# pablopalafox/semantic-depth

Hardware: AMD Instinct MI355X
Metric: fused frames/sec (FCN-8s+monodepth+pcl fusion) at 512x1024 (higher is better)
Workload: dtype fp32-grade: f32 operands as fp16 hi + 2^11-scaled lo planes (22 bits), 3 fp16 MFMA products, f32 accumulate; 1 GPU; BASELINE.json configs[3]: full fused pipeline (seg + depth + pcl back-projection + road width), batch 32 per GPU, 512x1024, monodepth-resnet50 on frame+flip, seeded synthetic weights; survey_config=4, engine=f16x2, approach=rw, overlap=True, full=False, found=32

## Files before the change

### semantic_depth_amd/csrc/dec_tail.hip

```cpp
#include "kernels.hpp"
#include "split_fmt.hpp"

namespace sd {

typedef float f32x4 __attribute__((ext_vector_type(4)));
typedef unsigned u32x4 __attribute__((ext_vector_type(4)));

constexpr int DT_TH = 8, DT_TW = 28;
constexpr int DT_AR = DT_TH / 2 + 4, DT_AC = 18, DT_APL = DT_AR * DT_AC * 4;
constexpr int DT_UR = DT_TH + 4, DT_UC = 34, DT_UPL = DT_UR * DT_UC * 2;
constexpr int DT_ER = DT_UR / 2, DT_EPL = DT_ER * DT_UC;
constexpr int DT_IR = DT_TH + 2, DT_IC = 32, DT_IPIX = 80;
constexpr int DT_DPL = DT_AR * DT_AC;
constexpr int DT_NG = 256;
constexpr int DT_NPIX = DT_TH * DT_TW;

template <bool HS>
__global__ __launch_bounds__(512, 1) void dec_tail1_kernel(const DecTailParams p) {
    constexpr int NPL = HS ? 2 : 3;
    constexpr int DT_UE = NPL * DT_UPL + NPL * DT_EPL;
    constexpr int DT_NA = (NPL * DT_APL + DT_NG - 1) / DT_NG, DT_ND = (NPL * DT_DPL + DT_NG - 1) / DT_NG, DT_NE = (NPL * DT_EPL + DT_NG - 1) / DT_NG;
    static_assert((2 * DT_UE + NPL * DT_APL) * 16 + DT_IR * DT_IC * DT_IPIX + NPL * DT_DPL * 4 <= 160 * 1024, "tiles fit the LDS of a CU");
    static_assert(DT_IR % 2 == 0 && DT_NPIX % 4 == 0 && DT_NPIX / 4 <= 64, "work split of stages 2 and 3");
    __shared__ __attribute__((aligned(16))) u32x4 UE[2 * DT_UE];
    __shared__ __attribute__((aligned(16))) u32x4 A[NPL * DT_APL];
    __shared__ __attribute__((aligned(16))) unsigned char I[DT_IR * DT_IC * DT_IPIX];
    __shared__ unsigned Dt[NPL * DT_DPL];
    const int t = threadIdx.x, lane = t & 63;
    const int wave = __builtin_amdgcn_readfirstlane(t >> 6);
    const bool s1 = wave < 4;
    const int wv = wave & 3, tg = t & (DT_NG - 1);
    const int H = p.H, W = p.W, Hs = H >> 1, Ws = W >> 1;
    const int ntx = (W + DT_TW - 1) / DT_TW, nty = H / DT_TH;
    const int ntiles = ntx * nty * p.N;
    const int lp = lane & 15, lg = lane >> 4;

    struct Tile { int img, y0, x0; };
    auto tile_of = [&](int it) {
        Tile r;
        const int tx = it % ntx; it /= ntx;
        r.x0 = tx * DT_TW < W - DT_TW ? tx * DT_TW : W - DT_TW;
        r.y0 = (it % nty) * DT_TH; r.img = it / nty;
        return r;
    };
    auto mac6 = [](const u32x4 (&w)[3], const u32x4& xh, const u32x4& xm, const u32x4& xl, f32x4 acc) {
        if constexpr (HS) {
            acc = mfma_frag16<true>(w[1], xh, acc);
            acc = mfma_frag16<true>(w[2], xm, acc);
            acc = mfma_frag16<true>(w[0], xh, acc);
            return acc;
        }
        acc = mfma_frag16<false>(w[2], xh, acc);
        acc = mfma_frag16<false>(w[1], xm, acc);
        acc = mfma_frag16<false>(w[0], xl, acc);
        acc = mfma_frag16<false>(w[1], xh, acc);
        acc = mfma_frag16<false>(w[0], xm, acc);
        acc = mfma_frag16<false>(w[0], xh, acc);
        return acc;
    };
    const float wdr0 = p.wd[lane], wdr1 = p.wd[64 + lane], wdr2 = p.wd[lane < 16 ? 128 + lane : 0];
    auto wd_at = [&](int i) {
        return __builtin_bit_cast(float, __builtin_amdgcn_readlane(__builtin_bit_cast(int, i < 64 ? wdr0 : i < 128 ? wdr1 : wdr2), i & 63));
    };
    auto head = [&](const Tile& tl, int pi) {
        const int ry = pi / DT_TW, cx = pi - ry * DT_TW;
        f32x4 v[3][4];
        auto tapload = [&](int slot, int tap) {
            const unsigned char* ip = I + ((ry + tap / 3) * DT_IC + cx + tap % 3) * DT_IPIX;
#pragma unroll
            for (int c4 = 0; c4 < 4; ++c4) v[slot][c4] = *reinterpret_cast<const f32x4*>(ip + 16 * c4);
        };
        tapload(0, 0); tapload(1, 1);
        float acc0 = p.bd[0], acc1 = 0.f;
#pragma unroll
        for (int tap = 0; tap < 9; ++tap) {
            if (tap + 2 < 9) tapload((tap + 2) % 3, tap + 2);
#pragma unroll
            for (int hf = 0; hf < 2; ++hf) {
                float w[8];
#pragma unroll
                for (int e = 0; e < 8; ++e) w[e] = wd_at(tap * 16 + 8 * hf + e);

#pragma unroll
                for (int e = 0; e < 8; e += 2) {
                    acc0 += v[tap % 3][2 * hf + (e >> 2)][e & 3] * w[e];
                    acc1 += v[tap % 3][2 * hf + ((e + 1) >> 2)][(e + 1) & 3] * w[e + 1];
                }

            }
        }
        const float acc = acc0 + acc1;
        p.out[((size_t)tl.img * H + tl.y0 + ry) * W + tl.x0 + cx] = 0.3f * (1.0f / (1.0f + expf(-acc)));
    };

    for (int i = t; i < 2 * DT_UE; i += 512) UE[i] = u32x4{0u, 0u, 0u, 0u};
    const int first = blockIdx.x, stride = gridDim.x;
    const int K = first < ntiles ? (ntiles - first + stride - 1) / stride : 0;

    if (s1) {
        int ga[DT_NA];
#pragma unroll
        for (int k = 0; k < DT_NA; ++k) {
            const int u = tg + DT_NG * k;
            const int pl = u / DT_APL, rem = u - pl * DT_APL, pix = rem >> 2, slot = rem & 3;
            const int arow = pix / DT_AC, acol = pix - arow * DT_AC;
            ga[k] = arow | (acol << 8) | ((slot ^ ((acol >> 1) & 3)) << 16) | (pl << 20) | ((u < NPL * DT_APL ? 1 : 0) << 24);
        }
        int gd[DT_ND];
#pragma unroll
        for (int k = 0; k < DT_ND; ++k) {
            const int d = tg + DT_NG * k;
            const int pl = d / DT_DPL, pix = d - pl * DT_DPL;
            const int arow = pix / DT_AC, acol = pix - arow * DT_AC;
            gd[k] = arow | (acol << 8) | (pl << 20) | ((d < NPL * DT_DPL ? 1 : 0) << 24);
        }
        int ge[DT_NE];
        int gew[DT_NE];
#pragma unroll
        for (int k = 0; k < DT_NE; ++k) {
            const int e = tg + DT_NG * k;
            const int pl = e / DT_EPL, pix = e - pl * DT_EPL;
            const int er = pix / DT_UC, uc = pix - er * DT_UC;
            auto dcol = [&](int dx) { int c = ((uc + dx) >> 1) + 1; return c < 0 ? 0 : c > DT_AC - 1 ? DT_AC - 1 : c; };
            ge[k] = er | (uc << 8) | (pl << 16) | ((e < NPL * DT_EPL ? 1 : 0) << 24);
            gew[k] = (pl * DT_DPL + (er + 1) * DT_AC + dcol(-1)) | ((dcol(0) - dcol(-1)) << 16) | ((dcol(1) - dcol(0)) << 17);
        }
        u32x4 pa[DT_NA];
        unsigned pd[DT_ND];
        auto prefetch = [&](const Tile& tl) {
            const int sy0 = (tl.y0 >> 1) - 2, sx0 = (tl.x0 >> 1) - 2;
            const uint16_t* const a = reinterpret_cast<const uint16_t*>(p.a);
            const uint16_t* const d2 = reinterpret_cast<const uint16_t*>(p.d2);
#pragma unroll
            for (int k = 0; k < DT_NA; ++k) {
                const int sy = sy0 + (ga[k] & 0xff), sx = sx0 + ((ga[k] >> 8) & 0xff);
                const bool ok = ((ga[k] >> 24) & 1) && (unsigned)sy < (unsigned)Hs && (unsigned)sx < (unsigned)Ws;
                const uint16_t* src = a + (size_t)((ga[k] >> 20) & 3) * p.a_plane + ((size_t)(tl.img * Hs + sy) * Ws + sx) * 32 + ((ga[k] >> 16) & 3) * 8;
                pa[k] = ok ? *reinterpret_cast<const u32x4*>(src) : u32x4{0u, 0u, 0u, 0u};
            }
#pragma unroll
            for (int k = 0; k < DT_ND; ++k) {
                const int sy = sy0 + (gd[k] & 0xff), sx = sx0 + ((gd[k] >> 8) & 0xff);
                const bool ok = ((gd[k] >> 24) & 1) && (unsigned)sy < (unsigned)Hs && (unsigned)sx < (unsigned)Ws;
                const uint16_t* src = d2 + (size_t)((gd[k] >> 20) & 3) * p.d_plane + ((size_t)(tl.img * Hs + sy) * Ws + sx) * 8;
                pd[k] = ok ? *reinterpret_cast<const unsigned*>(src) : 0u;
            }
        };
        auto stash = [&]() {
#pragma unroll
            for (int k = 0; k < DT_NA; ++k)
                if ((ga[k] >> 24) & 1) A[tg + DT_NG * k] = pa[k];
#pragma unroll
            for (int k = 0; k < DT_ND; ++k)
                if ((gd[k] >> 24) & 1) Dt[tg + DT_NG * k] = pd[k];
        };
        const int q = wv, py = q >> 1, px = q & 1;
        u32x4 w1[4][3];
#pragma unroll
        for (int tp = 0; tp < 4; ++tp) {
#pragma unroll
            for (int pl = 0; pl < NPL; ++pl) w1[tp][pl] = p.w1[((q * 4 + tp) * 3 + pl) * 64 + lane];
            if constexpr (HS) w1[tp][2] = hs_wscaled(w1[tp][0]);
        }
        const f32x4 bias1 = *reinterpret_cast<const f32x4*>(p.b1 + 4 * lg);

        Tile nxt = tile_of(K > 0 ? first : 0);
        if (K > 0) { prefetch(nxt); stash(); }
        __syncthreads();
        for (int k = 0; k <= K; ++k) {
            if (k < K) {
                const Tile cur = nxt;
                const int y0 = cur.y0, x0 = cur.x0;
                u32x4* const Ub = UE + (k & 1) * DT_UE;
                if (k + 1 < K) { nxt = tile_of(first + (k + 1) * stride); prefetch(nxt); }
#pragma unroll
                for (int j = 0; j < DT_NE; ++j) {
                    const int er = ge[j] & 0xff, uc = (ge[j] >> 8) & 0xff, pl = (ge[j] >> 16) & 3;
                    const int ys = (y0 >> 1) - 1 + er, x = x0 - 2 + uc;
                    const int wi = gew[j] & 0xffff, i0 = wi + ((gew[j] >> 16) & 1), i1 = i0 + ((gew[j] >> 17) & 1);
                    const unsigned a = Dt[wi], b0 = Dt[i0], c = Dt[i1];
                    const bool oky = (unsigned)ys < (unsigned)Hs;
                    u32x4 ev;
                    ev[0] = oky && (unsigned)(x - 1) < (unsigned)W ? a : 0u;
                    ev[1] = oky && (unsigned)x < (unsigned)W ? b0 : 0u;
                    ev[2] = oky && (unsigned)(x + 1) < (unsigned)W ? c : 0u;
                    ev[3] = 0u;
                    if ((ge[j] >> 24) & 1) Ub[NPL * DT_UPL + pl * DT_EPL + er * DT_UC + uc] = ev;
                }
                auto frag = [&](int r, int b, int pl) {
                    const int acol = lp + px + b;
                    return A[pl * DT_APL + (r * DT_AC + acol) * 4 + (lg ^ ((acol >> 1) & 3))];
                };
                u32x4 F[2][2][3];
#pragma unroll
                for (int b = 0; b < 2; ++b)
#pragma unroll
                    for (int pl = 0; pl < NPL; ++pl) F[0][b][pl] = frag(py, b, pl);
#pragma unroll
                for (int n = 0; n < DT_UR / 2; ++n) {
                    const int s0 = n & 1, s1_ = s0 ^ 1;
#pragma unroll
                    for (int b = 0; b < 2; ++b)
#pragma unroll
                        for (int pl = 0; pl < NPL; ++pl) F[s1_][b][pl] = frag(n + py + 1, b, pl);
                    f32x4 acc0 = {0.f, 0.f, 0.f, 0.f}, acc1 = {0.f, 0.f, 0.f, 0.f};
#pragma unroll
                    for (int b = 0; b < 2; ++b) {
                        acc0 = mac6(w1[b], F[s0][b][0], F[s0][b][1], F[s0][b][HS ? 1 : 2], acc0);
                        acc1 = mac6(w1[2 + b], F[s1_][b][0], F[s1_][b][1], F[s1_][b][HS ? 1 : 2], acc1);
                    }
                    f32x4 v = HS ? (acc0 + acc1) * p.alpha + bias1 : acc0 + acc1 + bias1;
                    v = act_split4<ACT_ELU>(v);
                    const int ru = 2 * n + py, uc = 2 * lp + px;
                    const bool in = (unsigned)(y0 - 2 + ru) < (unsigned)H && (unsigned)(x0 - 2 + uc) < (unsigned)W;
                    if (!in) v = f32x4{0.f, 0.f, 0.f, 0.f};
                    uint2 hh, mm, ll;
                    uint2* const up = reinterpret_cast<uint2*>(Ub) + ((ru * DT_UC + uc) * 2 + ((lg >> 1) ^ ((uc >> 2) & 1))) * 2 + (lg & 1);
                    if constexpr (HS) {
                        split4_hs(v, hh, mm, (sat_ptr_t) nullptr);
                        up[0] = hh; up[2 * DT_UPL] = mm;
                    } else {
                        split4_x3(v, hh, mm, ll);
                        up[0] = hh; up[2 * DT_UPL] = mm; up[4 * DT_UPL] = ll;
                    }
                }
            }
            __syncthreads();
            if (k + 1 < K) stash();
            __syncthreads();
        }
    } else {
        u32x4 w2[6][3];
#pragma unroll
        for (int ks = 0; ks < 6; ++ks) {
#pragma unroll
            for (int pl = 0; pl < NPL; ++pl) w2[ks][pl] = p.w2[(ks * 3 + pl) * 64 + lane];
            if constexpr (HS) w2[ks][2] = hs_wscaled(w2[ks][0]);
        }
        const f32x4 bias2 = *reinterpret_cast<const f32x4*>(p.b2 + 4 * lg);
        const int strip = wv & 1, ri0 = (DT_IR / 2) * (wv >> 1);
        const int c = 16 * strip + lp;
        const int uA = c + 1 + ((lg >> 1) - 1), uB = c + 2;
        const int offA = uA * 2 + ((lg & 1) ^ ((uA >> 2) & 1)), offB = uB * 2 + ((lg & 1) ^ ((uB >> 2) & 1));
        __syncthreads();
        for (int k = 0; k <= K; ++k) {
            const Tile cur = tile_of(first + (k >= 1 ? k - 1 : 0) * stride);
            if (k >= 1) {
                const u32x4* const Ub = UE + ((k - 1) & 1) * DT_UE;
                u32x4 G[3][2][3];
                auto gload = [&](int slot, int ru) {
#pragma unroll
                    for (int pl = 0; pl < NPL; ++pl) {
                        G[slot][0][pl] = Ub[pl * DT_UPL + ru * (DT_UC * 2) + offA];
                        G[slot][1][pl] = Ub[lg < 2 ? pl * DT_UPL + ru * (DT_UC * 2) + offB : NPL * DT_UPL + pl * DT_EPL + (ru >> 1) * DT_UC + c + 1];
                    }
                };
                gload(0, ri0); gload(1, ri0 + 1);
#pragma unroll
                for (int it = 0; it < DT_IR / 2; ++it) {
                    const int ri = ri0 + it;
                    gload((it + 2) % 3, ri + 2);
                    f32x4 acc[3];
#pragma unroll
                    for (int dy = 0; dy < 3; ++dy) {
                        acc[dy] = f32x4{0.f, 0.f, 0.f, 0.f};
                        const int sl = (it + dy) % 3;
                        acc[dy] = mac6(w2[2 * dy], G[sl][0][0], G[sl][0][1], G[sl][0][HS ? 1 : 2], acc[dy]);
                        acc[dy] = mac6(w2[2 * dy + 1], G[sl][1][0], G[sl][1][1], G[sl][1][HS ? 1 : 2], acc[dy]);
                    }
                    f32x4 v = HS ? ((acc[0] + acc[1]) + acc[2]) * p.alpha2 + bias2 : (acc[0] + acc[1]) + acc[2] + bias2;
                    v = act_split4<ACT_ELU>(v);
                    const bool in = (unsigned)(cur.y0 - 1 + ri) < (unsigned)H && (unsigned)(cur.x0 - 1 + c) < (unsigned)W;
                    if (!in) v = f32x4{0.f, 0.f, 0.f, 0.f};
                    *reinterpret_cast<f32x4*>(I + (ri * DT_IC + c) * DT_IPIX + 16 * lg) = v;
                }
            }
            __syncthreads();
            if (k >= 1 && lane < DT_NPIX / 4) head(cur, wv * (DT_NPIX / 4) + lane);
            __syncthreads();
        }
    }
}

bool dec_tail1_eligible(int H, int W) { return H % DT_TH == 0 && W % 2 == 0 && W >= DT_TW + 2; }

hipError_t launch_dec_tail1(const DecTailParams& p, hipStream_t s) {
    if (!dec_tail1_eligible(p.H, p.W)) return hipErrorInvalidValue;
    static int cus = 0;
    if (!cus) {
        int dev = 0;
        hipDeviceProp_t prop;
        if (hipGetDevice(&dev) != hipSuccess || hipGetDeviceProperties(&prop, dev) != hipSuccess) return hipErrorInvalidDevice;
        cus = prop.multiProcessorCount;
    }
    const int tiles = ((p.W + DT_TW - 1) / DT_TW) * (p.H / DT_TH) * p.N;
    const int wgs = cus - p.reserve_cus > 0 ? cus - p.reserve_cus : 1;
    const dim3 grid((unsigned)(tiles < wgs ? tiles : wgs));
    switch (p.scheme) {
        case SC_HS: hipLaunchKernelGGL(dec_tail1_kernel<true>, grid, dim3(512), 0, s, p); break;
        case SC_BF16X3: hipLaunchKernelGGL(dec_tail1_kernel<false>, grid, dim3(512), 0, s, p); break;
        default: return hipErrorInvalidValue;
    }
    return hipGetLastError();
}

}
```

Measured before the change: 436.8 frames/s.

## Use taller 12-row tiles for HS decoder tail with two-pixel head pass

Templates the decoder-tail kernel on tile height and uses 12-row tiles for the fp16 hi/lo split scheme, which lowers the share of halo rows recomputed per tile. Because a 12x28 tile exceeds one pixel per lane in the output head, a new head path has each lane compute two adjacent pixels. It keeps the head weights in registers and reads them with readlane, reusing the loaded input columns across both pixels. Tiles may now overhang the image bottom, so the head masks those rows. LDS use rises and there are fewer tiles to spread across CUs.

Result: no change. 438.8 frames/s, median of 6 (+0.5%).

```diff
diff --git a/semantic_depth_amd/csrc/dec_tail.hip b/semantic_depth_amd/csrc/dec_tail.hip
--- a/semantic_depth_amd/csrc/dec_tail.hip
+++ b/semantic_depth_amd/csrc/dec_tail.hip
@@ -4,24 +4,32 @@
 namespace sd {
 
 typedef float f32x4 __attribute__((ext_vector_type(4)));
+typedef float f32x2 __attribute__((ext_vector_type(2)));
 typedef unsigned u32x4 __attribute__((ext_vector_type(4)));
 
-constexpr int DT_TH = 8, DT_TW = 28;
-constexpr int DT_AR = DT_TH / 2 + 4, DT_AC = 18, DT_APL = DT_AR * DT_AC * 4;
-constexpr int DT_UR = DT_TH + 4, DT_UC = 34, DT_UPL = DT_UR * DT_UC * 2;
-constexpr int DT_ER = DT_UR / 2, DT_EPL = DT_ER * DT_UC;
-constexpr int DT_IR = DT_TH + 2, DT_IC = 32, DT_IPIX = 80;
-constexpr int DT_DPL = DT_AR * DT_AC;
+constexpr int DT_TW = 28;
+constexpr int DT_TH_HS = 12, DT_TH_X3 = 8;
+constexpr int DT_AC = 18;
+constexpr int DT_UC = 34;
+constexpr int DT_IC = 32, DT_IPIX = 80;
 constexpr int DT_NG = 256;
-constexpr int DT_NPIX = DT_TH * DT_TW;
-
-template <bool HS>
+
+template <bool HS, int TH>
 __global__ __launch_bounds__(512, 1) void dec_tail1_kernel(const DecTailParams p) {
     constexpr int NPL = HS ? 2 : 3;
+    constexpr int DT_TH = TH;
+    constexpr int DT_AR = DT_TH / 2 + 4, DT_APL = DT_AR * DT_AC * 4;
+    constexpr int DT_UR = DT_TH + 4, DT_UPL = DT_UR * DT_UC * 2;
+    constexpr int DT_ER = DT_UR / 2, DT_EPL = DT_ER * DT_UC;
+    constexpr int DT_IR = DT_TH + 2;
+    constexpr int DT_DPL = DT_AR * DT_AC;
+    constexpr int DT_NPIX = DT_TH * DT_TW;
+    constexpr bool DT_PAIRS = DT_NPIX / 4 > 64;
     constexpr int DT_UE = NPL * DT_UPL + NPL * DT_EPL;
     constexpr int DT_NA = (NPL * DT_APL + DT_NG - 1) / DT_NG, DT_ND = (NPL * DT_DPL + DT_NG - 1) / DT_NG, DT_NE = (NPL * DT_EPL + DT_NG - 1) / DT_NG;
     static_assert((2 * DT_UE + NPL * DT_APL) * 16 + DT_IR * DT_IC * DT_IPIX + NPL * DT_DPL * 4 <= 160 * 1024, "tiles fit the LDS of a CU");
-    static_assert(DT_IR % 2 == 0 && DT_NPIX % 4 == 0 && DT_NPIX / 4 <= 64, "work split of stages 2 and 3");
+    static_assert(DT_TH % 2 == 0 && DT_IR % 2 == 0 && DT_NPIX % 4 == 0, "work split of stages 1 and 2");
+    static_assert(DT_PAIRS ? DT_TH % 4 == 0 && DT_TW % 2 == 0 && DT_NPIX / 8 <= 64 : DT_TH == 8, "work split of stage 3 (8 rows: H % 8 == 0, no tile hangs over the image)");
     __shared__ __attribute__((aligned(16))) u32x4 UE[2 * DT_UE];
     __shared__ __attribute__((aligned(16))) u32x4 A[NPL * DT_APL];
     __shared__ __attribute__((aligned(16))) unsigned char I[DT_IR * DT_IC * DT_IPIX];
@@ -31,7 +39,7 @@
     const bool s1 = wave < 4;
     const int wv = wave & 3, tg = t & (DT_NG - 1);
     const int H = p.H, W = p.W, Hs = H >> 1, Ws = W >> 1;
-    const int ntx = (W + DT_TW - 1) / DT_TW, nty = H / DT_TH;
+    const int ntx = (W + DT_TW - 1) / DT_TW, nty = (H + DT_TH - 1) / DT_TH;
     const int ntiles = ntx * nty * p.N;
     const int lp = lane & 15, lg = lane >> 4;
 
@@ -91,6 +99,47 @@
         }
         const float acc = acc0 + acc1;
         p.out[((size_t)tl.img * H + tl.y0 + ry) * W + tl.x0 + cx] = 0.3f * (1.0f / (1.0f + expf(-acc)));
+    };
+
+    const float wr0 = p.wd[lane < 48 ? lane : 0], wr1 = p.wd[lane < 48 ? 48 + lane : 0], wr2 = p.wd[lane < 48 ? 96 + lane : 0];
+    auto head2 = [&](const Tile& tl, int ry, int cx, bool on) {
+        f32x2 acc[2] = {f32x2{p.bd[0], 0.f}, f32x2{p.bd[0], 0.f}};
+        float wa = wr0, wb = wr1, wc = wr2;
+        const unsigned char* ip = I + (ry * DT_IC + cx) * DT_IPIX;
+#pragma unroll 1
+        for (int dy = 0; dy < 3; ++dy) {
+            if (on) {
+                f32x4 v[4][4];
+#pragma unroll
+                for (int col = 0; col < 4; ++col)
+#pragma unroll
+                    for (int c4 = 0; c4 < 4; ++c4) v[col][c4] = *reinterpret_cast<const f32x4*>(ip + col * DT_IPIX + 16 * c4);
+#pragma unroll
+                for (int dx = 0; dx < 3; ++dx)
+#pragma unroll
+                    for (int hf = 0; hf < 2; ++hf) {
+                        float w[8];
+#pragma unroll
+                        for (int e = 0; e < 8; ++e) w[e] = __builtin_bit_cast(float, __builtin_amdgcn_readlane(__builtin_bit_cast(int, wa), dx * 16 + 8 * hf + e));
+#pragma unroll
+                        for (int e = 0; e < 8; e += 2) {
+                            const f32x2 ww = {w[e], w[e + 1]};
+#pragma unroll
+                            for (int j = 0; j < 2; ++j) {
+                                const f32x4 vv = v[dx + j][2 * hf + (e >> 2)];
+                                acc[j] += ((e & 2) ? f32x2{vv[2], vv[3]} : f32x2{vv[0], vv[1]}) * ww;
+                            }
+                        }
+                    }
+            }
+            ip += DT_IC * DT_IPIX;
+            const float wt = wa; wa = wb; wb = wc; wc = wt;
+        }
+        if (on) {
+#pragma unroll
+            for (int j = 0; j < 2; ++j)
+                p.out[((size_t)tl.img * H + tl.y0 + ry) * W + tl.x0 + cx + j] = 0.3f * (1.0f / (1.0f + expf(-(acc[j][0] + acc[j][1]))));
+        }
     };
 
     for (int i = t; i < 2 * DT_UE; i += 512) UE[i] = u32x4{0u, 0u, 0u, 0u};
@@ -276,13 +325,18 @@
                 }
             }
             __syncthreads();
-            if (k >= 1 && lane < DT_NPIX / 4) head(cur, wv * (DT_NPIX / 4) + lane);
+            if constexpr (!DT_PAIRS) {
+                if (k >= 1 && lane < DT_NPIX / 4) head(cur, wv * (DT_NPIX / 4) + lane);
+            } else if (k >= 1) {
+                const int r3 = lane / (DT_TW / 2), ry = wv * (DT_TH / 4) + r3, cx = 2 * (lane - r3 * (DT_TW / 2));
+                head2(cur, ry, cx, lane < DT_NPIX / 8 && cur.y0 + ry < H);
+            }
             __syncthreads();
         }
     }
 }
 
-bool dec_tail1_eligible(int H, int W) { return H % DT_TH == 0 && W % 2 == 0 && W >= DT_TW + 2; }
+bool dec_tail1_eligible(int H, int W) { return H % 8 == 0 && W % 2 == 0 && W >= DT_TW + 2; }
 
 hipError_t launch_dec_tail1(const DecTailParams& p, hipStream_t s) {
     if (!dec_tail1_eligible(p.H, p.W)) return hipErrorInvalidValue;
@@ -293,14 +347,13 @@
         if (hipGetDevice(&dev) != hipSuccess || hipGetDeviceProperties(&prop, dev) != hipSuccess) return hipErrorInvalidDevice;
         cus = prop.multiProcessorCount;
     }
-    const int tiles = ((p.W + DT_TW - 1) / DT_TW) * (p.H / DT_TH) * p.N;
+    if (p.scheme != SC_HS && p.scheme != SC_BF16X3) return hipErrorInvalidValue;
+    const int th = p.scheme == SC_HS ? DT_TH_HS : DT_TH_X3;
+    const int tiles = ((p.W + DT_TW - 1) / DT_TW) * ((p.H + th - 1) / th) * p.N;
     const int wgs = cus - p.reserve_cus > 0 ? cus - p.reserve_cus : 1;
     const dim3 grid((unsigned)(tiles < wgs ? tiles : wgs));
-    switch (p.scheme) {
-        case SC_HS: hipLaunchKernelGGL(dec_tail1_kernel<true>, grid, dim3(512), 0, s, p); break;
-        case SC_BF16X3: hipLaunchKernelGGL(dec_tail1_kernel<false>, grid, dim3(512), 0, s, p); break;
-        default: return hipErrorInvalidValue;
-    }
+    if (p.scheme == SC_HS) hipLaunchKernelGGL((dec_tail1_kernel<true, DT_TH_HS>), grid, dim3(512), 0, s, p);
+    else hipLaunchKernelGGL((dec_tail1_kernel<false, DT_TH_X3>), grid, dim3(512), 0, s, p);
     return hipGetLastError();
 }
 
```
